# DCDmllm/AnyEdit

Hardware: NVIDIA H100
Metric: edited images/sec (512x512, 50-step DDIM, CFG) (higher is better)
Workload: dtype f16

## Files before the change

anyedit_b200/csrc/gemm_wgmma.cu:

```cuda
#include <cuda.h>
#include <stdlib.h>

#include "common.cuh"
#include "wgmma.cuh"

namespace anysd {

constexpr int G_BM = 128, G_BK = 64, G_THREADS = 384;
constexpr int G_A_BYTES = G_BM * G_BK * 2;

template <int BN>
struct GCfg {
    static constexpr int STAGE_BYTES = G_A_BYTES + BN * G_BK * 2;
    static constexpr int RED_BYTES = 8 * BN * 8;
    static constexpr int PAR_BYTES = 2 * 2 * BN * 4;
    static constexpr int FIT = (212 * 1024 - RED_BYTES - PAR_BYTES) / STAGE_BYTES;
    static constexpr int STAGES = FIT > 6 ? 6 : FIT;
    static constexpr int SMEM = STAGES * STAGE_BYTES + RED_BYTES + PAR_BYTES + 1024 + 256;
};

struct GArgs {
    const float* bias;
    const float* rowadd;
    const __half* residual;
    void* out;
    int M, N, ldo, ldr, ld_rowadd, rows_per_batch;
    int act, out_f16;
    int num_kb, tiles_m, tiles_n, num_tiles;
    int Nimg, Ho, Wo;
    int BW, BH, NB, tiles_w, tiles_h;
    int kb_per_tap, stride;
    int pad_lo;
    float* stats;
    int stats_hw, stats_spi, stats_nimg;
    int splits, kb_per_split, num_units;
    float* sk_ws;
    unsigned int* sk_cnt;
    float* row_stats;
    const float* ln_stats;
    const float* ln_colsum;
    int ln_slabs;
    float ln_eps, ln_inv_k;
};

__device__ __forceinline__ void g_bar_init(uint32_t bar, uint32_t count) {
    asm volatile("mbarrier.init.shared::cta.b64 [%0], %1;" ::"r"(bar), "r"(count));
}
__device__ __forceinline__ void g_expect_tx(uint32_t bar, uint32_t bytes) {
    asm volatile("mbarrier.arrive.expect_tx.shared::cta.b64 _, [%0], %1;" ::"r"(bar), "r"(bytes) : "memory");
}
__device__ __forceinline__ void g_arrive(uint32_t bar) {
    asm volatile("mbarrier.arrive.shared::cta.b64 _, [%0];" ::"r"(bar) : "memory");
}
__device__ __forceinline__ void g_wait(uint32_t bar, uint32_t parity) {
    asm volatile(
        "{\n\t"
        ".reg .pred P1;\n\t"
        "WAIT_LOOP:\n\t"
        "mbarrier.try_wait.parity.shared::cta.b64 P1, [%0], %1;\n\t"
        "@P1 bra DONE;\n\t"
        "bra WAIT_LOOP;\n\t"
        "DONE:\n\t"
        "}" ::"r"(bar), "r"(parity) : "memory");
}
__device__ __forceinline__ void g_tma_2d(uint32_t dst, const CUtensorMap* tm, uint32_t bar, int c0, int c1) {
    asm volatile("cp.async.bulk.tensor.2d.shared::cluster.global.mbarrier::complete_tx::bytes [%0], [%1, {%3, %4}], [%2];"
                 ::"r"(dst), "l"(tm), "r"(bar), "r"(c0), "r"(c1) : "memory");
}
__device__ __forceinline__ void g_tma_4d(uint32_t dst, const CUtensorMap* tm, uint32_t bar, int c0, int c1, int c2, int c3) {
    asm volatile("cp.async.bulk.tensor.4d.shared::cluster.global.mbarrier::complete_tx::bytes [%0], [%1, {%3, %4, %5, %6}], [%2];"
                 ::"r"(dst), "l"(tm), "r"(bar), "r"(c0), "r"(c1), "r"(c2), "r"(c3) : "memory");
}
__device__ __forceinline__ void g_pair_bar(int id) { asm volatile("bar.sync %0, 64;" ::"r"(id) : "memory"); }
__device__ __forceinline__ void g_wg_bar(int id) { asm volatile("bar.sync %0, 128;" ::"r"(id) : "memory"); }

__device__ __forceinline__ float p_gelu(float v) {
    const float t = fminf(v * v, 36.0f);
    float q = fmaf(t, 2.483638929e-05f, 7.36060983e-04f);
    q = fmaf(q, t, -0.10598272654f);
    q = fmaf(q, t, -2.30164716054f);
    float e, r;
    asm("ex2.approx.ftz.f32 %0, %1;" : "=f"(e) : "f"(v * q));
    asm("rcp.approx.ftz.f32 %0, %1;" : "=f"(r) : "f"(1.0f + e));
    return v * r;
}

struct TileCoord {
    int nt;
    int m0;
    int tw, th, tn;
};

template <bool CONV>
__device__ __forceinline__ TileCoord tile_coord(const GArgs& p, int tile) {
    TileCoord c;
    const int mt = tile / p.tiles_n;
    c.nt = tile - mt * p.tiles_n;
    c.m0 = mt * G_BM;
    c.tw = c.th = c.tn = 0;
    if (CONV) {
        c.tw = mt % p.tiles_w;
        c.th = (mt / p.tiles_w) % p.tiles_h;
        c.tn = mt / (p.tiles_w * p.tiles_h);
    }
    return c;
}

template <int BN, bool CONV>
__global__ void __launch_bounds__(G_THREADS, 1)
gemm_wgmma_kernel(const __grid_constant__ CUtensorMap tmA, const __grid_constant__ CUtensorMap tmB, const GArgs p) {
    using Cfg = GCfg<BN>;
    constexpr int STAGES = Cfg::STAGES;
    extern __shared__ unsigned char g_smem_raw[];
    const uint32_t raw = smem_u32(g_smem_raw);
    const uint32_t base = (raw + 1023u) & ~1023u;
    unsigned char* smem = g_smem_raw + (base - raw);
    float2* red = reinterpret_cast<float2*>(smem + STAGES * Cfg::STAGE_BYTES);
    float* par = reinterpret_cast<float*>(smem + STAGES * Cfg::STAGE_BYTES + Cfg::RED_BYTES);
    const uint32_t bars = base + STAGES * Cfg::STAGE_BYTES + Cfg::RED_BYTES + Cfg::PAR_BYTES;
    volatile int* sk_flag = reinterpret_cast<volatile int*>(smem + STAGES * Cfg::STAGE_BYTES + Cfg::RED_BYTES + Cfg::PAR_BYTES + 16 * STAGES);
    auto full_bar = [&](int s) { return bars + 8u * s; };
    auto empty_bar = [&](int s) { return bars + 8u * (STAGES + s); };
    const int warp = threadIdx.x >> 5, lane = threadIdx.x & 31;

    if (threadIdx.x == 0) {
        asm volatile("prefetch.tensormap [%0];" ::"l"(&tmA) : "memory");
        asm volatile("prefetch.tensormap [%0];" ::"l"(&tmB) : "memory");
        for (int s = 0; s < STAGES; ++s) {
            g_bar_init(full_bar(s), 1);
            g_bar_init(empty_bar(s), 8);
        }
        asm volatile("fence.mbarrier_init.release.cluster;" ::: "memory");
    }
    __syncthreads();

    if (warp < 4) {
        asm volatile("setmaxnreg.dec.sync.aligned.u32 40;" ::: "memory");
        if (warp == 0 && lane == 0) {
            uint32_t g = 0;
            for (int unit = blockIdx.x; unit < p.num_units; unit += gridDim.x) {
                const int tile = unit / p.splits;
                const int kb0 = (unit - tile * p.splits) * p.kb_per_split;
                const int kb1 = kb0 + p.kb_per_split < p.num_kb ? kb0 + p.kb_per_split : p.num_kb;
                const TileCoord c = tile_coord<CONV>(p, tile);
                const int n0 = c.nt * BN;
                for (int kb = kb0; kb < kb1; ++kb, ++g) {
                    const int s = g % STAGES;
                    g_wait(empty_bar(s), ((g / STAGES) & 1) ^ 1);
                    const uint32_t sa = base + s * Cfg::STAGE_BYTES, sb = sa + G_A_BYTES;
                    g_expect_tx(full_bar(s), Cfg::STAGE_BYTES);
                    if (CONV) {
                        const int tap = kb / p.kb_per_tap;
                        const int c0 = (kb - tap * p.kb_per_tap) * G_BK;
                        const int ky = tap / 3, kx = tap - ky * 3;
                        g_tma_4d(sa, &tmA, full_bar(s), c0, c.tw * p.BW * p.stride + kx - p.pad_lo,
                                 c.th * p.BH * p.stride + ky - p.pad_lo, c.tn * p.NB);
                    } else {
                        g_tma_2d(sa, &tmA, full_bar(s), kb * G_BK, c.m0);
                    }
                    g_tma_2d(sb, &tmB, full_bar(s), kb * G_BK, n0);
                }
            }
        }
        return;
    }

    asm volatile("setmaxnreg.inc.sync.aligned.u32 232;" ::: "memory");
    const int wg = (warp >> 2) - 1;
    const int wq = warp & 3;
    const int ew = wg * 4 + wq;
    const int slab = ew >> 1;
    const int rl0 = wg * 64 + wq * 16 + (lane >> 2);
    const int q4 = lane & 3;
    const bool ln_in = !CONV && p.ln_stats != nullptr;
    const bool row_st = !CONV && p.row_stats != nullptr;
    float* s_bias = par + wg * 2 * BN;
    float* s_cs = s_bias + BN;
    const int wtid = threadIdx.x & 127;
    float acc[BN / 2];
    uint32_t g = 0;
    for (int unit = blockIdx.x; unit < p.num_units; unit += gridDim.x) {
        const int tile = unit / p.splits;
        const int kb0 = (unit - tile * p.splits) * p.kb_per_split;
        const int kb1 = kb0 + p.kb_per_split < p.num_kb ? kb0 + p.kb_per_split : p.num_kb;
        const TileCoord c = tile_coord<CONV>(p, tile);
        const int n0 = c.nt * BN;
        float pb[2], pc[2];
#pragma unroll
        for (int r = 0; r < 2; ++r) {
            const int j = wtid + 128 * r, col = n0 + j;
            pb[r] = (j < BN && col < p.N && p.bias != nullptr) ? __ldg(p.bias + col) : 0.f;
            pc[r] = (j < BN && col < p.N && ln_in) ? __ldg(p.ln_colsum + col) : 0.f;
        }
#pragma unroll
        for (int i = 0; i < BN / 2; ++i) acc[i] = 0.f;
        for (int kb = kb0; kb < kb1; ++kb, ++g) {
            const int s = g % STAGES;
            g_wait(full_bar(s), (g / STAGES) & 1);
            const uint32_t sa = base + s * Cfg::STAGE_BYTES + wg * 64 * 128, sb = base + s * Cfg::STAGE_BYTES + G_A_BYTES;
            wg_fence();
#pragma unroll
            for (int k = 0; k < G_BK / 16; ++k) Wgmma<BN>::ss(acc, wg_desc(sa + 32 * k, 16, 1024), wg_desc(sb + 32 * k, 16, 1024), 1);
            wg_commit();
            wg_wait<1>();
            if (kb > kb0) {
                __syncwarp();
                if (lane == 0) g_arrive(empty_bar((g - 1) % STAGES));
            }
        }
        wg_wait<0>();
#pragma unroll
        for (int i = 0; i < BN / 2; ++i) wg_fence_regs(acc[i]);
        if (kb1 > kb0) {
            __syncwarp();
            if (lane == 0) g_arrive(empty_bar((g - 1) % STAGES));
        }
        g_wg_bar(5 + wg);
#pragma unroll
        for (int r = 0; r < 2; ++r) {
            if (wtid + 128 * r < BN) {
                s_bias[wtid + 128 * r] = pb[r];
                s_cs[wtid + 128 * r] = pc[r];
            }
        }
        g_wg_bar(5 + wg);

        if (p.splits > 1) {
            const int ks = unit - tile * p.splits;
            const float* wst = p.sk_ws + (size_t)tile * p.splits * (G_BM * BN);
            float* mine = p.sk_ws + ((size_t)tile * p.splits + ks) * (G_BM * BN);
#pragma unroll
            for (int i = 0; i < BN / 8; ++i)
#pragma unroll
                for (int h = 0; h < 2; ++h)
                    __stcg(reinterpret_cast<float2*>(mine + (size_t)(rl0 + 8 * h) * BN + 8 * i + 2 * q4),
                           make_float2(acc[4 * i + 2 * h], acc[4 * i + 2 * h + 1]));
            __threadfence();
            g_pair_bar(1 + slab);
            if ((ew & 1) == 0 && lane == 0) {
                unsigned int* cnt = p.sk_cnt + (size_t)tile * 4 + slab;
                const unsigned int old = atomicAdd(cnt, 1u);
                if (old == (unsigned)p.splits - 1) *cnt = 0;
                sk_flag[slab] = old == (unsigned)p.splits - 1;
            }
            g_pair_bar(1 + slab);
            const bool last = sk_flag[slab] != 0;
            g_pair_bar(1 + slab);
            if (!last) continue;
            __threadfence();
#pragma unroll
            for (int i = 0; i < BN / 2; ++i) acc[i] = 0.f;
            for (int k2 = 0; k2 < p.splits; ++k2) {
#pragma unroll
                for (int i = 0; i < BN / 8; ++i)
#pragma unroll
                    for (int h = 0; h < 2; ++h) {
                        const float2 f = __ldcg(reinterpret_cast<const float2*>(wst + (size_t)k2 * (G_BM * BN) +
                                                                                 (size_t)(rl0 + 8 * h) * BN + 8 * i + 2 * q4));
                        acc[4 * i + 2 * h] += f.x;
                        acc[4 * i + 2 * h + 1] += f.y;
                    }
            }
        }

        size_t pix[2];
        bool valid[2];
        int img[2];
        float ln_nm[2] = {0.f, 0.f}, ln_rs[2] = {1.f, 1.f};
#pragma unroll
        for (int h = 0; h < 2; ++h) {
            const int r = rl0 + 8 * h;
            if (CONV) {
                const int x = r % p.BW, y = (r / p.BW) % p.BH, n = r / (p.BW * p.BH);
                const int X = c.tw * p.BW + x, Y = c.th * p.BH + y, I = c.tn * p.NB + n;
                valid[h] = X < p.Wo && Y < p.Ho && I < p.Nimg;
                pix[h] = ((size_t)I * p.Ho + Y) * p.Wo + X;
                img[h] = I < p.Nimg ? I : p.Nimg - 1;
            } else {
                const int m = c.m0 + r;
                valid[h] = m < p.M;
                pix[h] = (size_t)m;
                img[h] = (m < p.M ? m : p.M - 1) / p.rows_per_batch;
                if (ln_in) {
                    const float2* sp2 = reinterpret_cast<const float2*>(p.ln_stats) + (m < p.M ? m : p.M - 1);
                    float s1 = 0.f, s2 = 0.f;
                    for (int sl = 0; sl < p.ln_slabs; ++sl) {
                        const float2 f = __ldg(sp2 + (size_t)sl * p.M);
                        s1 += f.x;
                        s2 += f.y;
                    }
                    const double mean = (double)s1 * (double)p.ln_inv_k;
                    double var = (double)s2 * (double)p.ln_inv_k - mean * mean;
                    if (var < 0.0) var = 0.0;
                    ln_nm[h] = -(float)mean;
                    ln_rs[h] = rsqrtf((float)var + p.ln_eps);
                }
            }
        }
        auto store2 = [&](int h, int ocol, float a, float b) {
            if (valid[h]) {
                if (p.residual != nullptr) {
                    const float2 r = __half22float2(*reinterpret_cast<const __half2*>(p.residual + pix[h] * p.ldr + ocol));
                    a += r.x;
                    b += r.y;
                }
                if (p.out_f16) *reinterpret_cast<__half2*>((__half*)p.out + pix[h] * p.ldo + ocol) = __floats2half2_rn(a, b);
                else *reinterpret_cast<float2*>((float*)p.out + pix[h] * p.ldo + ocol) = make_float2(a, b);
            }
        };

        float rs1[2] = {0.f, 0.f}, rs2[2] = {0.f, 0.f};
        constexpr int CH = 4;
        constexpr int UNROLL = BN <= 64 ? BN / 8 / CH : 1;
#pragma unroll UNROLL
        for (int i0 = 0; i0 < BN / 8; i0 += CH) {
            if (n0 + 8 * i0 >= p.N) break;
            float a[CH][4];
#pragma unroll
            for (int u = 0; u < CH; ++u)
#pragma unroll
                for (int e = 0; e < 4; ++e) a[u][e] = acc[4 * u + e];
#pragma unroll
            for (int k = CH; k < BN / 8; k += CH)
#pragma unroll
                for (int u = 0; u < CH; ++u)
#pragma unroll
                    for (int e = 0; e < 4; ++e) a[u][e] = k == i0 ? acc[4 * (k + u) + e] : a[u][e];
            float2 ra[CH][2];
            __half2 rr[CH][2];
#pragma unroll
            for (int u = 0; u < CH; ++u) {
                const int cw = n0 + 8 * (i0 + u) + 2 * q4;
                const bool in = cw < p.N;
#pragma unroll
                for (int h = 0; h < 2; ++h) {
                    ra[u][h] = (in && p.rowadd != nullptr)
                                   ? __ldg(reinterpret_cast<const float2*>(p.rowadd + (size_t)img[h] * p.ld_rowadd + cw))
                                   : make_float2(0.f, 0.f);
                    rr[u][h] = (in && valid[h] && p.residual != nullptr && p.act != 2)
                                   ? *reinterpret_cast<const __half2*>(p.residual + pix[h] * p.ldr + cw)
                                   : __floats2half2_rn(0.f, 0.f);
                }
            }
#pragma unroll
        for (int u = 0; u < CH; ++u) {
            const int i = i0 + u;
            if (n0 + 8 * i >= p.N) break;
            const int col = n0 + 8 * i + 2 * q4;
            float v[2][2];
            const float2 bb = *reinterpret_cast<const float2*>(s_bias + 8 * i + 2 * q4);
            if (ln_in) {
                const float2 cs = *reinterpret_cast<const float2*>(s_cs + 8 * i + 2 * q4);
#pragma unroll
                for (int h = 0; h < 2; ++h) {
                    v[h][0] = fmaf(ln_rs[h], fmaf(ln_nm[h], cs.x, a[u][2 * h]), bb.x);
                    v[h][1] = fmaf(ln_rs[h], fmaf(ln_nm[h], cs.y, a[u][2 * h + 1]), bb.y);
                }
            } else {
#pragma unroll
                for (int h = 0; h < 2; ++h) {
                    v[h][0] = a[u][2 * h] + bb.x;
                    v[h][1] = a[u][2 * h + 1] + bb.y;
                }
            }
#pragma unroll
            for (int h = 0; h < 2; ++h) {
                v[h][0] += ra[u][h].x;
                v[h][1] += ra[u][h].y;
            }
            if (p.act == 2) {
                float gv[2];
#pragma unroll
                for (int h = 0; h < 2; ++h) gv[h] = v[h][0] * (p.out_f16 ? p_gelu(v[h][1]) : gelu_erf_f(v[h][1]));
                const float recv = __shfl_xor_sync(0xffffffffu, (lane & 1) ? gv[0] : gv[1], 1);
                const int h = lane & 1;
                const int ocol = (col >> 1) - h;
                if (h) store2(1, ocol, recv, gv[1]);
                else store2(0, ocol, gv[0], recv);
                continue;
            }
            if (p.act != 0) {
#pragma unroll
                for (int h = 0; h < 2; ++h)
#pragma unroll
                    for (int e = 0; e < 2; ++e)
                        v[h][e] = p.act == 1 ? silu_f(v[h][e])
                                             : (p.act == 3 ? (p.out_f16 ? p_gelu(v[h][e]) : gelu_erf_f(v[h][e])) : quick_gelu_f(v[h][e]));
            }
#pragma unroll
            for (int h = 0; h < 2; ++h) {
                const float2 r = __half22float2(rr[u][h]);
                v[h][0] += r.x;
                v[h][1] += r.y;
                if (valid[h]) {
                    if (p.out_f16) *reinterpret_cast<__half2*>((__half*)p.out + pix[h] * p.ldo + col) = __floats2half2_rn(v[h][0], v[h][1]);
                    else *reinterpret_cast<float2*>((float*)p.out + pix[h] * p.ldo + col) = make_float2(v[h][0], v[h][1]);
                }
            }
            if (p.stats != nullptr) {
                float a0 = v[0][0] + v[1][0], a1 = v[0][1] + v[1][1];
                float b0 = v[0][0] * v[0][0] + v[1][0] * v[1][0], b1 = v[0][1] * v[0][1] + v[1][1] * v[1][1];
#pragma unroll
                for (int o = 4; o < 32; o <<= 1) {
                    a0 += __shfl_xor_sync(0xffffffffu, a0, o);
                    a1 += __shfl_xor_sync(0xffffffffu, a1, o);
                    b0 += __shfl_xor_sync(0xffffffffu, b0, o);
                    b1 += __shfl_xor_sync(0xffffffffu, b1, o);
                }
                if (lane < 4) {
                    red[ew * BN + 8 * i + 2 * lane] = make_float2(a0, b0);
                    red[ew * BN + 8 * i + 2 * lane + 1] = make_float2(a1, b1);
                }
            }
            if (row_st) {
#pragma unroll
                for (int h = 0; h < 2; ++h) {
                    rs1[h] += v[h][0] + v[h][1];
                    rs2[h] = fmaf(v[h][0], v[h][0], fmaf(v[h][1], v[h][1], rs2[h]));
                }
                if ((i & 7) == 7) {
#pragma unroll
                    for (int h = 0; h < 2; ++h) {
                        rs1[h] += __shfl_xor_sync(0xffffffffu, rs1[h], 1);
                        rs2[h] += __shfl_xor_sync(0xffffffffu, rs2[h], 1);
                        rs1[h] += __shfl_xor_sync(0xffffffffu, rs1[h], 2);
                        rs2[h] += __shfl_xor_sync(0xffffffffu, rs2[h], 2);
                        if (q4 == 0 && valid[h])
                            reinterpret_cast<float2*>(p.row_stats)[(size_t)((n0 >> 6) + (i >> 3)) * p.M + pix[h]] =
                                make_float2(rs1[h], rs2[h]);
                        rs1[h] = rs2[h] = 0.f;
                    }
                }
            }
        }
        }
        if (p.stats != nullptr) {
            g_pair_bar(1 + slab);
            if ((ew & 1) == 0) {
                int simg, sii;
                if (CONV) {
                    const int ppi = p.BW * p.BH;
                    simg = c.tn * p.NB + (slab * 32) / ppi;
                    sii = (c.th * p.tiles_w + c.tw) * (ppi >> 5) + (((slab * 32) % ppi) >> 5);
                } else {
                    const int r0 = c.m0 + slab * 32;
                    simg = r0 / p.stats_hw;
                    sii = (r0 - simg * p.stats_hw) >> 5;
                    if (r0 >= p.M) simg = p.stats_nimg;
                }
                if (simg < p.stats_nimg) {
                    for (int j = lane; j < BN && n0 + j < p.N; j += 32) {
                        const float2 x0 = red[ew * BN + j], x1 = red[(ew + 1) * BN + j];
                        reinterpret_cast<float2*>(p.stats)[((size_t)simg * p.stats_spi + sii) * p.N + n0 + j] =
                            make_float2(x0.x + x1.x, x0.y + x1.y);
                    }
                }
            }
            g_pair_bar(1 + slab);
        }
    }
}

typedef CUresult (*EncodeTiledFnP)(CUtensorMap*, CUtensorMapDataType, cuuint32_t, void*, const cuuint64_t*,
                                   const cuuint64_t*, const cuuint32_t*, const cuuint32_t*, CUtensorMapInterleave,
                                   CUtensorMapSwizzle, CUtensorMapL2promotion, CUtensorMapFloatOOBfill);
static EncodeTiledFnP p_get_encode() {
    static EncodeTiledFnP fn = nullptr;
    static bool tried = false;
    if (!tried) {
        tried = true;
        void* f = nullptr;
        cudaDriverEntryPointQueryResult qr;
        if (cudaGetDriverEntryPoint("cuTensorMapEncodeTiled", &f, cudaEnableDefault, &qr) == cudaSuccess &&
            qr == cudaDriverEntryPointSuccess)
            fn = (EncodeTiledFnP)f;
    }
    return fn;
}

struct PMapKey {
    const void* ptr;
    uint64_t d0, d1, d2, d3, ld;
    uint32_t b0, b1, b2, b3, es, rank;
    bool operator==(const PMapKey& o) const {
        return ptr == o.ptr && d0 == o.d0 && d1 == o.d1 && d2 == o.d2 && d3 == o.d3 && ld == o.ld && b0 == o.b0 && b1 == o.b1 &&
               b2 == o.b2 && b3 == o.b3 && es == o.es && rank == o.rank;
    }
};
struct PMapSlot {
    PMapKey key;
    CUtensorMap map;
    bool valid;
};
constexpr int P_MAP_SLOTS = 4096;
static thread_local PMapSlot* p_map_table = nullptr;
static PMapSlot* p_map_slot(const PMapKey& k) {
    if (p_map_table == nullptr) p_map_table = (PMapSlot*)calloc(P_MAP_SLOTS, sizeof(PMapSlot));
    uint64_t h = (uint64_t)(uintptr_t)k.ptr * 0x9E3779B97F4A7C15ull;
    h ^= (k.d0 * 31 + k.d1) * 0xC2B2AE3D27D4EB4Full + (k.d2 * 131 + k.d3 * 17 + k.ld) * 0x165667B19E3779F9ull;
    h ^= ((uint64_t)k.b0 << 40) ^ ((uint64_t)k.b1 << 28) ^ ((uint64_t)k.b2 << 16) ^ ((uint64_t)k.b3 << 4) ^ k.es ^ ((uint64_t)k.rank << 60);
    return p_map_table ? &p_map_table[(h >> 20) % P_MAP_SLOTS] : nullptr;
}

static bool p_map_2d(CUtensorMap* tm, const void* ptr, uint64_t inner, uint64_t outer, uint64_t ld, uint32_t bi, uint32_t bo) {
    const PMapKey key = {ptr, inner, outer, 0, 0, ld, bi, bo, 0, 0, 1, 2};
    PMapSlot* slot = p_map_slot(key);
    if (slot && slot->valid && slot->key == key) {
        *tm = slot->map;
        return true;
    }
    cuuint64_t dims[2] = {inner, outer};
    cuuint64_t strides[1] = {ld * 2};
    cuuint32_t box[2] = {bi, bo};
    cuuint32_t es[2] = {1, 1};
    const bool ok = p_get_encode()(tm, CU_TENSOR_MAP_DATA_TYPE_FLOAT16, 2, const_cast<void*>(ptr), dims, strides, box, es,
                                   CU_TENSOR_MAP_INTERLEAVE_NONE, CU_TENSOR_MAP_SWIZZLE_128B, CU_TENSOR_MAP_L2_PROMOTION_L2_256B,
                                   CU_TENSOR_MAP_FLOAT_OOB_FILL_NONE) == CUDA_SUCCESS;
    if (ok && slot) {
        slot->key = key;
        slot->map = *tm;
        slot->valid = true;
    }
    return ok;
}
static bool p_map_nhwc(CUtensorMap* tm, const void* ptr, int N, int H, int W, int C, int ld, int BW, int BH, int NB, int s) {
    const PMapKey key = {ptr, (uint64_t)C, (uint64_t)W, (uint64_t)H, (uint64_t)N, (uint64_t)ld, 64u, (uint32_t)BW, (uint32_t)BH, (uint32_t)NB,
                         (uint32_t)s, 4};
    PMapSlot* slot = p_map_slot(key);
    if (slot && slot->valid && slot->key == key) {
        *tm = slot->map;
        return true;
    }
    cuuint64_t dims[4] = {(cuuint64_t)C, (cuuint64_t)W, (cuuint64_t)H, (cuuint64_t)N};
    cuuint64_t strides[3] = {(cuuint64_t)ld * 2, (cuuint64_t)W * ld * 2, (cuuint64_t)H * W * ld * 2};
    cuuint32_t box[4] = {64u, (cuuint32_t)(BW * s), (cuuint32_t)(BH * s), (cuuint32_t)NB};
    cuuint32_t es[4] = {1, (cuuint32_t)s, (cuuint32_t)s, 1};
    const bool ok = p_get_encode()(tm, CU_TENSOR_MAP_DATA_TYPE_FLOAT16, 4, const_cast<void*>(ptr), dims, strides, box, es,
                                   CU_TENSOR_MAP_INTERLEAVE_NONE, CU_TENSOR_MAP_SWIZZLE_128B, CU_TENSOR_MAP_L2_PROMOTION_L2_256B,
                                   CU_TENSOR_MAP_FLOAT_OOB_FILL_NONE) == CUDA_SUCCESS;
    if (ok && slot) {
        slot->key = key;
        slot->map = *tm;
        slot->valid = true;
    }
    return ok;
}

static int p_pow2_ceil(int v) {
    int r = 1;
    while (r < v) r <<= 1;
    return r;
}
static int p_pick_extent(int len, int cap) {
    int lim = p_pow2_ceil(len);
    if (lim > cap) lim = cap;
    for (int c = lim; c >= 4; c >>= 1)
        if (len % c == 0) return c;
    return lim;
}

__global__ void upsample2x_kernel(const uint4* __restrict__ src, uint4* __restrict__ dst, int H, int W, int CV, long long total) {
    for (long long i = blockIdx.x * (long long)blockDim.x + threadIdx.x; i < total; i += (long long)gridDim.x * blockDim.x) {
        const int cv = (int)(i % CV);
        long long r = i / CV;
        const int ox = (int)(r % (2 * W));
        r /= (2 * W);
        const int oy = (int)(r % (2 * H));
        const long long n = r / (2 * H);
        dst[i] = __ldg(src + ((n * H + (oy >> 1)) * W + (ox >> 1)) * CV + cv);
    }
}

int launch_upsample2x(const __half* src, __half* dst, int N, int H, int W, int C, cudaStream_t st) {
    const long long total = (long long)N * 4 * H * W * (C / 8);
    int grid = (int)((total + 255) / 256);
    if (grid > sm_count() * 16) grid = sm_count() * 16;
    upsample2x_kernel<<<grid, 256, 0, st>>>((const uint4*)src, (uint4*)dst, H, W, C / 8, total);
    return check_launch("upsample2x");
}

static void p_conv_patch(const anysd_gemm_params* q, int* Ho, int* Wo, int* BW, int* BH, int* NB) {
    const int Hin = q->H << q->upsample, Win = q->Wd << q->upsample;
    *Ho = q->conv_pad ? (Hin - 2) / 2 + 1 : (Hin - 1) / q->stride + 1;
    *Wo = q->conv_pad ? (Win - 2) / 2 + 1 : (Win - 1) / q->stride + 1;
    *BW = p_pick_extent(*Wo, 128);
    *BH = p_pick_extent(*Ho, 128 / *BW);
    *NB = 128 / (*BW * *BH);
}

int wg_stats_slabs(const anysd_gemm_params* q) {
    if (q->act == 2 || q->out_dtype != ANYSD_F16) return 0;
    const int hw = q->rows_per_batch;
    if (hw <= 0 || hw % 32 != 0 || q->M % hw != 0) return 0;
    if (q->conv) {
        int Ho, Wo, BW, BH, NB;
        p_conv_patch(q, &Ho, &Wo, &BW, &BH, &NB);
        if (Ho * Wo != hw || (BW * BH) % 32 != 0 || Wo % BW != 0 || Ho % BH != 0) return 0;
    }
    return hw / 32;
}

static int p_geometry_splits(const anysd_gemm_params* q, int num_kb) {
    static const char* force_sk = getenv("ANYSD_GEMM_SPLITK");
    if (q->act == 2 || q->out_dtype != ANYSD_F16 || q->row_stats != nullptr || q->ln_stats != nullptr) return 1;
    int rows_per_image = q->rows_per_batch;
    if (q->conv) {
        int Ho, Wo, BW, BH, NB;
        p_conv_patch(q, &Ho, &Wo, &BW, &BH, &NB);
        rows_per_image = Ho * Wo;
    }
    if (rows_per_image <= 0 || rows_per_image > G_BM) return 1;
    if (force_sk) {
        const int f = atoi(force_sk);
        return (f <= 1 || num_kb / f < 8) ? 1 : (f > 8 ? 8 : f);
    }
    return (q->conv && num_kb >= 256) ? 3 : 1;
}

static void p_select(const anysd_gemm_params* q, int tiles_m, int num_kb, int* bn_out, int* splits_out) {
    static const char* force_bn = getenv("ANYSD_GEMM_BN");
    const int sp = splits_out ? p_geometry_splits(q, num_kb) : 1;
    int bn = 256;
    double best = -1;
    static const int widths[4] = {256, 192, 128, 64};
    for (int wi = 0; wi < 4; ++wi) {
        const int w = widths[wi];
        if (force_bn && atoi(force_bn) != w) continue;
        const long units = (long)tiles_m * cdiv(q->N, w) * sp;
        const long slots = sm_count();
        const long rounds = (units + slots - 1) / slots;
        const double cost = (double)rounds * (w + 270) * ((double)cdiv(num_kb, sp) + (sp > 1 ? 8.0 : 0.0));
        if (best < 0 || cost < best) { best = cost; bn = w; }
    }
    *bn_out = bn;
    if (splits_out) *splits_out = sp;
}
static size_t p_splitk_bytes(int tiles_m, int N, int bn, int splits) {
    if (splits <= 1) return 0;
    return (size_t)tiles_m * cdiv(N, bn) * splits * G_BM * bn * sizeof(float);
}

static void p_tiles(const anysd_gemm_params* q, int* tiles_m, int* num_kb) {
    if (q->conv) {
        int Ho, Wo, BW, BH, NB;
        p_conv_patch(q, &Ho, &Wo, &BW, &BH, &NB);
        *tiles_m = cdiv(Wo, BW) * cdiv(Ho, BH) * cdiv(q->Nimg, NB);
        *num_kb = 9 * (q->Cin / G_BK);
    } else {
        *tiles_m = cdiv(q->M, G_BM);
        *num_kb = cdiv(q->K, G_BK);
    }
}

size_t wg_splitk_bytes(const anysd_gemm_params* q) {
    int tiles_m, num_kb, bn, splits;
    p_tiles(q, &tiles_m, &num_kb);
    p_select(q, tiles_m, num_kb, &bn, &splits);
    return p_splitk_bytes(tiles_m, q->N, bn, splits);
}

static const char* wg_ln_unsupported(const anysd_gemm_params* q) {
    if (q->conv) return "dense contractions only";
    if (q->out_dtype != ANYSD_F16) return "fp16 output only";
    if (q->row_stats != nullptr) {
        if (q->act != 0) return "row statistics need act = 0";
        if (q->N % 64 != 0) return "row statistics need N % 64 == 0";
        if ((uintptr_t)q->row_stats % 8) return "row_stats must be 8-byte aligned";
    }
    if (q->ln_stats != nullptr) {
        if (q->K % 64 != 0) return "folded LayerNorm needs K % 64 == 0";
        if (q->bias == nullptr || q->ln_colsum == nullptr) return "folded LayerNorm needs bias (beta W^T + b) and ln_colsum";
        if (((uintptr_t)q->ln_stats % 8) || ((uintptr_t)q->ln_colsum % 16)) return "ln_stats / ln_colsum misaligned";
        if (q->N % 32 != 0) return "folded LayerNorm needs N % 32 == 0";
        if (q->act != 0 && q->act != 1 && q->act != 2) return "folded LayerNorm: act must be 0, 1 or 2";
    }
    return nullptr;
}

bool wg_supported(const anysd_gemm_params* q) {
    if (q->N % 8 != 0 || q->K % 8 != 0) return false;
    if (q->act == 2 && q->N % 16 != 0) return false;
    const int n_out = q->act == 2 ? q->N / 2 : q->N;
    if (((uintptr_t)q->out % 16) || q->ldo % 8 != 0 || n_out % 4 != 0) return false;
    if (q->residual && (((uintptr_t)q->residual % 16) || q->ldr % 8 != 0)) return false;
    if (q->bias && ((uintptr_t)q->bias % 16)) return false;
    if (q->rowadd && (((uintptr_t)q->rowadd % 16) || q->ld_rowadd % 4 != 0)) return false;
    if (q->conv) {
        if (q->Cin % G_BK != 0) return false;
        if (q->upsample) {
            const size_t need = (size_t)q->Nimg * (2 * q->H) * (2 * q->Wd) * q->Cin * sizeof(__half);
            if (q->workspace == nullptr || q->workspace_bytes < need || ((uintptr_t)q->workspace % 16)) return false;
        }
    }
    return p_get_encode() != nullptr;
}

template <int BN, bool CONV>
static int p_launch(const CUtensorMap& tmA, const CUtensorMap& tmB, const GArgs& a, cudaStream_t st) {
    static bool done[64];
    int dev = 0;
    cudaGetDevice(&dev);
    dev &= 63;
    if (!done[dev]) {
        cudaError_t e = cudaFuncSetAttribute(gemm_wgmma_kernel<BN, CONV>, cudaFuncAttributeMaxDynamicSharedMemorySize, GCfg<BN>::SMEM);
        if (e != cudaSuccess) {
            set_error("wgmma gemm: smem opt-in failed: %s", cudaGetErrorString(e));
            return ANYSD_ECUDA;
        }
        done[dev] = true;
    }
    int grid = sm_count();
    if (grid > a.num_units) grid = a.num_units;
    gemm_wgmma_kernel<BN, CONV><<<grid, G_THREADS, GCfg<BN>::SMEM, st>>>(tmA, tmB, a);
    return check_launch(CONV ? "conv3x3 (wgmma)" : "gemm (wgmma)");
}

template <bool CONV>
static int p_launch_bn(int bn, const CUtensorMap& tmA, const CUtensorMap& tmB, const GArgs& a, cudaStream_t st) {
    switch (bn) {
        case 256: return p_launch<256, CONV>(tmA, tmB, a, st);
        case 192: return p_launch<192, CONV>(tmA, tmB, a, st);
        case 128: return p_launch<128, CONV>(tmA, tmB, a, st);
        default: return p_launch<64, CONV>(tmA, tmB, a, st);
    }
}

int launch_gemm_wg(const anysd_gemm_params* q, cudaStream_t st) {
    GArgs a;
    a.stats = nullptr;
    a.stats_hw = a.stats_spi = a.stats_nimg = 0;
    if (q->stats != nullptr) {
        a.stats_spi = wg_stats_slabs(q);
        if (a.stats_spi == 0 || q->stats_images <= 0) {
            set_error("gemm: output statistics requested for a shape that cannot produce them (M=%d rows_per_batch=%d conv=%d act=%d); "
                      "query anysd_gemm_stats_slabs first", q->M, q->rows_per_batch, q->conv, q->act);
            return ANYSD_EUNSUPPORTED;
        }
        a.stats = q->stats;
        a.stats_hw = q->rows_per_batch;
        a.stats_nimg = q->stats_images;
    }
    a.row_stats = q->row_stats;
    a.ln_stats = q->ln_stats;
    a.ln_colsum = q->ln_colsum;
    a.ln_slabs = q->K / 64;
    a.ln_eps = q->ln_eps;
    a.ln_inv_k = 1.0f / (float)q->K;
    if (q->row_stats != nullptr || q->ln_stats != nullptr) {
        const char* why = wg_ln_unsupported(q);
        if (why) {
            set_error("gemm: LayerNorm fold / row statistics: %s (M=%d N=%d K=%d act=%d)", why, q->M, q->N, q->K, q->act);
            return ANYSD_EUNSUPPORTED;
        }
        if (q->stats != nullptr || q->act >= 3) {
            set_error("gemm: LayerNorm fold / row statistics cannot be combined with GroupNorm statistics or GELU epilogues");
            return ANYSD_EUNSUPPORTED;
        }
    }
    a.bias = q->bias;
    a.rowadd = q->rowadd;
    a.residual = (const __half*)q->residual;
    a.out = q->out;
    a.M = q->M;
    a.N = q->N;
    a.ldo = q->ldo;
    a.ldr = q->ldr;
    a.ld_rowadd = q->ld_rowadd;
    a.rows_per_batch = q->rows_per_batch > 0 ? q->rows_per_batch : 1;
    a.act = q->act;
    a.out_f16 = q->out_dtype == ANYSD_F16;
    a.Nimg = q->Nimg;
    a.BW = a.BH = a.NB = a.tiles_w = a.tiles_h = 1;
    a.kb_per_tap = 1;
    a.stride = q->conv ? q->stride : 1;
    a.pad_lo = (q->conv && q->conv_pad) ? 0 : 1;
    a.Ho = a.Wo = 0;
    CUtensorMap tmA, tmB;
    bool ok = true;
    p_tiles(q, &a.tiles_m, &a.num_kb);
    if (q->conv) {
        const void* img = q->A;
        int Hin = q->H, Win = q->Wd;
        if (q->upsample) {
            int rc = launch_upsample2x((const __half*)q->A, (__half*)q->workspace, q->Nimg, q->H, q->Wd, q->Cin, st);
            if (rc) return rc;
            img = q->workspace;
            Hin *= 2;
            Win *= 2;
        }
        p_conv_patch(q, &a.Ho, &a.Wo, &a.BW, &a.BH, &a.NB);
        a.tiles_w = cdiv(a.Wo, a.BW);
        a.tiles_h = cdiv(a.Ho, a.BH);
        a.kb_per_tap = q->Cin / G_BK;
        ok = ok && p_map_nhwc(&tmA, img, q->Nimg, Hin, Win, q->Cin, q->Cin, a.BW, a.BH, a.NB, a.stride);
    } else {
        ok = ok && p_map_2d(&tmA, q->A, (uint64_t)q->K, (uint64_t)q->M, (uint64_t)q->lda, G_BK, G_BM);
    }
    int bn = 256, splits = 1;
    p_select(q, a.tiles_m, a.num_kb, &bn, &splits);
    const size_t sk_need = p_splitk_bytes(a.tiles_m, q->N, bn, splits);
    if (splits > 1 && (q->splitk_workspace == nullptr || q->splitk_workspace_bytes < sk_need || q->splitk_counters == nullptr ||
                       (size_t)a.tiles_m * cdiv(q->N, bn) * 4 * sizeof(unsigned int) > q->splitk_counters_bytes)) {
        splits = 1;
        p_select(q, a.tiles_m, a.num_kb, &bn, nullptr);
    }
    a.tiles_n = cdiv(q->N, bn);
    ok = ok && p_map_2d(&tmB, q->W, (uint64_t)q->K, (uint64_t)q->N, (uint64_t)q->ldw, G_BK, bn);
    if (!ok) {
        set_error("wgmma gemm: cuTensorMapEncodeTiled failed (M=%d N=%d K=%d conv=%d)", q->M, q->N, q->K, q->conv);
        return ANYSD_ECUDA;
    }
    a.num_tiles = a.tiles_m * a.tiles_n;
    a.splits = splits;
    a.kb_per_split = cdiv(a.num_kb, splits);
    a.num_units = a.num_tiles * splits;
    a.sk_ws = (float*)q->splitk_workspace;
    a.sk_cnt = (unsigned int*)q->splitk_counters;
    return q->conv ? p_launch_bn<true>(bn, tmA, tmB, a, st) : p_launch_bn<false>(bn, tmA, tmB, a, st);
}

}
```

Measured before the change: 3.634.

## Add ping-pong warpgroup GEMM kernel for short-K non-conv GEMMs

Adds a 128x128 ping-pong kernel in which two consumer warpgroups take alternate tiles and hand off the MMA turn through named barriers. Each warpgroup's epilogue, which stages output through per-warp shared memory with coalesced 16-byte stores and cp.async residual loads, overlaps the other warpgroup's mainloop. The selector routes non-conv GEMMs with at most 10 K-blocks and at least two tiles per SM to this kernel. The aim is to hide epilogue cost on short-K GEMMs, at the cost of more complexity and a larger shared-memory footprint that may reduce pipeline stages.

```diff
diff --git a/anyedit_b200/csrc/gemm_wgmma.cu b/anyedit_b200/csrc/gemm_wgmma.cu
--- a/anyedit_b200/csrc/gemm_wgmma.cu
+++ b/anyedit_b200/csrc/gemm_wgmma.cu
@@ -8,15 +8,19 @@
 
 constexpr int G_BM = 128, G_BK = 64, G_THREADS = 384;
 constexpr int G_A_BYTES = G_BM * G_BK * 2;
+constexpr int G_OUT_PITCH_MAX = 160, G_RES_PITCH = 80;
+constexpr int G_STG_WARP = 16 * G_OUT_PITCH_MAX + 16 * G_RES_PITCH + 16 * 8;
 
 template <int BN>
-struct GCfg {
+struct GPingCfg {
+    static_assert(BN == 128, "ping-pong tiles are 128 x 128");
     static constexpr int STAGE_BYTES = G_A_BYTES + BN * G_BK * 2;
     static constexpr int RED_BYTES = 8 * BN * 8;
     static constexpr int PAR_BYTES = 2 * 2 * BN * 4;
-    static constexpr int FIT = (212 * 1024 - RED_BYTES - PAR_BYTES) / STAGE_BYTES;
+    static constexpr int STG_BYTES = 8 * G_STG_WARP;
+    static constexpr int FIT = (212 * 1024 - RED_BYTES - PAR_BYTES - STG_BYTES) / STAGE_BYTES;
     static constexpr int STAGES = FIT > 6 ? 6 : FIT;
-    static constexpr int SMEM = STAGES * STAGE_BYTES + RED_BYTES + PAR_BYTES + 1024 + 256;
+    static constexpr int SMEM = STAGES * STAGE_BYTES + RED_BYTES + PAR_BYTES + STG_BYTES + 1024 + 256;
 };
 
 struct GArgs {
@@ -73,6 +77,8 @@
 }
 __device__ __forceinline__ void g_pair_bar(int id) { asm volatile("bar.sync %0, 64;" ::"r"(id) : "memory"); }
 __device__ __forceinline__ void g_wg_bar(int id) { asm volatile("bar.sync %0, 128;" ::"r"(id) : "memory"); }
+__device__ __forceinline__ void g_turn_wait(int id) { asm volatile("bar.sync %0, 256;" ::"r"(id) : "memory"); }
+__device__ __forceinline__ void g_turn_pass(int id) { asm volatile("bar.arrive %0, 256;" ::"r"(id) : "memory"); }
 
 __device__ __forceinline__ float p_gelu(float v) {
     const float t = fminf(v * v, 36.0f);
@@ -106,10 +112,26 @@
     return c;
 }
 
+__device__ __forceinline__ void unit_kb(const GArgs& p, int unit, int& tile, int& kb0, int& kb1) {
+    tile = unit / p.splits;
+    kb0 = (unit - tile * p.splits) * p.kb_per_split;
+    kb1 = kb0 + p.kb_per_split < p.num_kb ? kb0 + p.kb_per_split : p.num_kb;
+}
+
+template <int BN>
+struct GCoopCfg {
+    static constexpr int STAGE_BYTES = G_A_BYTES + BN * G_BK * 2;
+    static constexpr int RED_BYTES = 8 * BN * 8;
+    static constexpr int PAR_BYTES = 2 * 2 * BN * 4;
+    static constexpr int FIT = (212 * 1024 - RED_BYTES - PAR_BYTES) / STAGE_BYTES;
+    static constexpr int STAGES = FIT > 6 ? 6 : FIT;
+    static constexpr int SMEM = STAGES * STAGE_BYTES + RED_BYTES + PAR_BYTES + 1024 + 256;
+};
+
 template <int BN, bool CONV>
 __global__ void __launch_bounds__(G_THREADS, 1)
-gemm_wgmma_kernel(const __grid_constant__ CUtensorMap tmA, const __grid_constant__ CUtensorMap tmB, const GArgs p) {
-    using Cfg = GCfg<BN>;
+gemm_coop_kernel(const __grid_constant__ CUtensorMap tmA, const __grid_constant__ CUtensorMap tmB, const GArgs p) {
+    using Cfg = GCoopCfg<BN>;
     constexpr int STAGES = Cfg::STAGES;
     extern __shared__ unsigned char g_smem_raw[];
     const uint32_t raw = smem_u32(g_smem_raw);
@@ -461,6 +483,369 @@
     }
 }
 
+template <int BN, bool CONV>
+__global__ void __launch_bounds__(G_THREADS, 1)
+gemm_pingpong_kernel(const __grid_constant__ CUtensorMap tmA, const __grid_constant__ CUtensorMap tmB, const GArgs p) {
+    using Cfg = GPingCfg<BN>;
+    constexpr int STAGES = Cfg::STAGES;
+    extern __shared__ unsigned char g_smem_raw[];
+    const uint32_t raw = smem_u32(g_smem_raw);
+    const uint32_t base = (raw + 1023u) & ~1023u;
+    unsigned char* smem = g_smem_raw + (base - raw);
+    unsigned char* tail = smem + STAGES * Cfg::STAGE_BYTES;
+    float2* red = reinterpret_cast<float2*>(tail);
+    float* par = reinterpret_cast<float*>(tail + Cfg::RED_BYTES);
+    unsigned char* stg = tail + Cfg::RED_BYTES + Cfg::PAR_BYTES;
+    const uint32_t bars = base + STAGES * Cfg::STAGE_BYTES + Cfg::RED_BYTES + Cfg::PAR_BYTES + Cfg::STG_BYTES;
+        auto full_bar = [&](int s) { return bars + 8u * s; };
+    auto empty_bar = [&](int s) { return bars + 8u * (STAGES + s); };
+    const int warp = threadIdx.x >> 5, lane = threadIdx.x & 31;
+
+    if (threadIdx.x == 0) {
+        asm volatile("prefetch.tensormap [%0];" ::"l"(&tmA) : "memory");
+        asm volatile("prefetch.tensormap [%0];" ::"l"(&tmB) : "memory");
+        for (int s = 0; s < STAGES; ++s) {
+            g_bar_init(full_bar(s), 1);
+            g_bar_init(empty_bar(s), 4);
+        }
+        asm volatile("fence.mbarrier_init.release.cluster;" ::: "memory");
+    }
+    __syncthreads();
+
+    if (warp < 4) {
+        asm volatile("setmaxnreg.dec.sync.aligned.u32 40;" ::: "memory");
+        if (warp == 0 && lane == 0) {
+            uint32_t g = 0;
+            for (int unit = blockIdx.x; unit < p.num_units; unit += gridDim.x) {
+                int tile, kb0, kb1;
+                unit_kb(p, unit, tile, kb0, kb1);
+                const TileCoord c = tile_coord<CONV>(p, tile);
+                const int n0 = c.nt * BN;
+                for (int kb = kb0; kb < kb1; ++kb, ++g) {
+                    const int s = g % STAGES;
+                    g_wait(empty_bar(s), ((g / STAGES) & 1) ^ 1);
+                    const uint32_t sa = base + s * Cfg::STAGE_BYTES, sb = sa + G_A_BYTES;
+                    g_expect_tx(full_bar(s), Cfg::STAGE_BYTES);
+                    if (CONV) {
+                        const int tap = kb / p.kb_per_tap;
+                        const int c0 = (kb - tap * p.kb_per_tap) * G_BK;
+                        const int ky = tap / 3, kx = tap - ky * 3;
+                        g_tma_4d(sa, &tmA, full_bar(s), c0, c.tw * p.BW * p.stride + kx - p.pad_lo,
+                                 c.th * p.BH * p.stride + ky - p.pad_lo, c.tn * p.NB);
+                    } else {
+                        g_tma_2d(sa, &tmA, full_bar(s), kb * G_BK, c.m0);
+                    }
+                    g_tma_2d(sb, &tmB, full_bar(s), kb * G_BK, n0);
+                }
+            }
+        }
+        return;
+    }
+
+    asm volatile("setmaxnreg.inc.sync.aligned.u32 232;" ::: "memory");
+    const int wg = (warp >> 2) - 1;
+    const int wq = warp & 3;
+    const int ew = wg * 4 + wq;
+    const int pair = 1 + 2 * wg + (wq >> 1);
+    const int q4 = lane & 3;
+    const bool ln_in = !CONV && p.ln_stats != nullptr;
+    const bool row_st = !CONV && p.row_stats != nullptr;
+    const bool geglu = p.act == 2;
+    const int n_out = geglu ? p.N >> 1 : p.N;
+    const int oes = p.out_f16 ? 2 : 4;
+    const int opitch = p.out_f16 ? 144 : 160;
+    float* s_bias = par + wg * 2 * BN;
+    float* s_cs = s_bias + BN;
+    unsigned char* s_out = stg + ew * G_STG_WARP;
+    __half* s_res = reinterpret_cast<__half*>(s_out + 16 * G_OUT_PITCH_MAX);
+    long long* s_pix = reinterpret_cast<long long*>(s_out + 16 * G_OUT_PITCH_MAX + 16 * G_RES_PITCH);
+    const int wtid = threadIdx.x & 127;
+    float acc[BN];
+    uint32_t g = 0;
+    if (wg == 1) {
+        int tile, kb0, kb1;
+        unit_kb(p, blockIdx.x, tile, kb0, kb1);
+        g += kb1 - kb0;
+    }
+    for (int unit = blockIdx.x + wg * gridDim.x; unit < p.num_units; unit += 2 * gridDim.x) {
+        int tile, kb0, kb1;
+        unit_kb(p, unit, tile, kb0, kb1);
+        const TileCoord c = tile_coord<CONV>(p, tile);
+        const int n0 = c.nt * BN;
+        float pb[2], pc[2];
+#pragma unroll
+        for (int r = 0; r < 2; ++r) {
+            const int j = wtid + 128 * r, col = n0 + j;
+            pb[r] = (j < BN && col < p.N && p.bias != nullptr) ? __ldg(p.bias + col) : 0.f;
+            pc[r] = (j < BN && col < p.N && ln_in) ? __ldg(p.ln_colsum + col) : 0.f;
+        }
+#pragma unroll
+        for (int i = 0; i < BN; ++i) acc[i] = 0.f;
+        if (unit != (int)blockIdx.x) g_turn_wait(7 + wg);
+        for (int kb = kb0; kb < kb1; ++kb, ++g) {
+            const int s = g % STAGES;
+            g_wait(full_bar(s), (g / STAGES) & 1);
+            const uint32_t sa = base + s * Cfg::STAGE_BYTES, sb = sa + G_A_BYTES;
+            wg_fence();
+#pragma unroll
+            for (int k = 0; k < G_BK / 16; ++k)
+#pragma unroll
+                for (int h2 = 0; h2 < 2; ++h2)
+                    Wgmma<BN>::ss(acc + h2 * (BN / 2), wg_desc(sa + h2 * 64 * 128 + 32 * k, 16, 1024), wg_desc(sb + 32 * k, 16, 1024), 1);
+            wg_commit();
+            wg_wait<1>();
+            if (kb > kb0) {
+                __syncwarp();
+                if (lane == 0) g_arrive(empty_bar((g - 1) % STAGES));
+            }
+        }
+        const uint32_t g_last = g - 1;
+        if (unit + (int)gridDim.x < p.num_units) {
+            g_turn_pass(7 + (wg ^ 1));
+            int t2, k0, k1;
+            unit_kb(p, unit + gridDim.x, t2, k0, k1);
+            g += k1 - k0;
+        }
+        wg_wait<0>();
+#pragma unroll
+        for (int i = 0; i < BN; ++i) wg_fence_regs(acc[i]);
+        if (kb1 > kb0) {
+            __syncwarp();
+            if (lane == 0) g_arrive(empty_bar(g_last % STAGES));
+        }
+        g_wg_bar(5 + wg);
+#pragma unroll
+        for (int r = 0; r < 2; ++r) {
+            if (wtid + 128 * r < BN) {
+                s_bias[wtid + 128 * r] = pb[r];
+                s_cs[wtid + 128 * r] = pc[r];
+            }
+        }
+        g_wg_bar(5 + wg);
+
+#pragma unroll 1
+        for (int h2 = 0; h2 < 2; ++h2) {
+            const int rl0 = 64 * h2 + 16 * wq + (lane >> 2);
+            size_t pix[2];
+            bool valid[2];
+            int img[2];
+            float ln_nm[2] = {0.f, 0.f}, ln_rs[2] = {1.f, 1.f};
+#pragma unroll
+            for (int h = 0; h < 2; ++h) {
+                const int r = rl0 + 8 * h;
+                if (CONV) {
+                    const int x = r % p.BW, y = (r / p.BW) % p.BH, n = r / (p.BW * p.BH);
+                    const int X = c.tw * p.BW + x, Y = c.th * p.BH + y, I = c.tn * p.NB + n;
+                    valid[h] = X < p.Wo && Y < p.Ho && I < p.Nimg;
+                    pix[h] = ((size_t)I * p.Ho + Y) * p.Wo + X;
+                    img[h] = I < p.Nimg ? I : p.Nimg - 1;
+                } else {
+                    const int m = c.m0 + r;
+                    valid[h] = m < p.M;
+                    pix[h] = (size_t)m;
+                    img[h] = (m < p.M ? m : p.M - 1) / p.rows_per_batch;
+                    if (ln_in) {
+                        const float2* sp2 = reinterpret_cast<const float2*>(p.ln_stats) + (m < p.M ? m : p.M - 1);
+                        float s1 = 0.f, s2 = 0.f;
+                        for (int sl = 0; sl < p.ln_slabs; ++sl) {
+                            const float2 f = __ldg(sp2 + (size_t)sl * p.M);
+                            s1 += f.x;
+                            s2 += f.y;
+                        }
+                        const double mean = (double)s1 * (double)p.ln_inv_k;
+                        double var = (double)s2 * (double)p.ln_inv_k - mean * mean;
+                        if (var < 0.0) var = 0.0;
+                        ln_nm[h] = -(float)mean;
+                        ln_rs[h] = rsqrtf((float)var + p.ln_eps);
+                    }
+                }
+            }
+            if (q4 == 0) {
+                s_pix[lane >> 2] = valid[0] ? (long long)pix[0] : -1ll;
+                s_pix[(lane >> 2) + 8] = valid[1] ? (long long)pix[1] : -1ll;
+            }
+            __syncwarp();
+
+            float rs1[2] = {0.f, 0.f}, rs2[2] = {0.f, 0.f};
+            constexpr int CH = 4;
+            constexpr int UNROLL = BN <= 64 ? BN / 8 / CH : 1;
+#pragma unroll UNROLL
+            for (int i0 = 0; i0 < BN / 8; i0 += CH) {
+                if (n0 + 8 * i0 >= p.N) break;
+                const int ob = geglu ? (n0 + 8 * i0) >> 1 : n0 + 8 * i0;
+                if (p.residual != nullptr) {
+                    const int rsh = geglu ? 1 : 2;
+#pragma unroll
+                    for (int t2 = 0; t2 < 2; ++t2) {
+                        const int t = lane + 32 * t2, r = t >> rsh, vi = t & ((1 << rsh) - 1), oc = ob + 8 * vi;
+                        if (r < 16) {
+                            const long long px = s_pix[r];
+                            const bool in = px >= 0 && oc < n_out;
+                            cp_async16(smem_u32(s_res + r * (G_RES_PITCH / 2) + 8 * vi),
+                                       in ? p.residual + (size_t)px * p.ldr + oc : p.residual, in);
+                        }
+                    }
+                    cp_async_commit();
+                }
+                float a[CH][4];
+                const int kk = h2 * (BN / 8) + i0;
+#pragma unroll
+                for (int u = 0; u < CH; ++u)
+#pragma unroll
+                    for (int e = 0; e < 4; ++e) a[u][e] = acc[4 * u + e];
+#pragma unroll
+                for (int k = CH; k < BN / 4; k += CH)
+#pragma unroll
+                    for (int u = 0; u < CH; ++u)
+#pragma unroll
+                        for (int e = 0; e < 4; ++e) a[u][e] = k == kk ? acc[4 * (k + u) + e] : a[u][e];
+                if (p.residual != nullptr) {
+                    cp_async_wait<0>();
+                    __syncwarp();
+                }
+                auto put = [&](int h, int oc, float x, float y) {
+                    const int r = (lane >> 2) + 8 * h;
+                    if (p.residual != nullptr) {
+                        const float2 rr = __half22float2(*reinterpret_cast<const __half2*>(s_res + r * (G_RES_PITCH / 2) + oc));
+                        x += rr.x;
+                        y += rr.y;
+                    }
+                    if (p.out_f16) *reinterpret_cast<__half2*>(s_out + r * opitch + 2 * oc) = __floats2half2_rn(x, y);
+                    else *reinterpret_cast<float2*>(s_out + r * opitch + 4 * oc) = make_float2(x, y);
+                    return make_float2(x, y);
+                };
+#pragma unroll
+                for (int u = 0; u < CH; ++u) {
+                    const int i = i0 + u;
+                    if (n0 + 8 * i >= p.N) break;
+                    float v[2][2];
+                    const float2 bb = *reinterpret_cast<const float2*>(s_bias + 8 * i + 2 * q4);
+                    if (ln_in) {
+                        const float2 cs = *reinterpret_cast<const float2*>(s_cs + 8 * i + 2 * q4);
+#pragma unroll
+                        for (int h = 0; h < 2; ++h) {
+                            v[h][0] = fmaf(ln_rs[h], fmaf(ln_nm[h], cs.x, a[u][2 * h]), bb.x);
+                            v[h][1] = fmaf(ln_rs[h], fmaf(ln_nm[h], cs.y, a[u][2 * h + 1]), bb.y);
+                        }
+                    } else {
+#pragma unroll
+                        for (int h = 0; h < 2; ++h) {
+                            v[h][0] = a[u][2 * h] + bb.x;
+                            v[h][1] = a[u][2 * h + 1] + bb.y;
+                        }
+                    }
+                    if (p.rowadd != nullptr) {
+#pragma unroll
+                        for (int h = 0; h < 2; ++h) {
+                            const float2 ra = __ldg(reinterpret_cast<const float2*>(p.rowadd + (size_t)img[h] * p.ld_rowadd + n0 + 8 * i + 2 * q4));
+                            v[h][0] += ra.x;
+                            v[h][1] += ra.y;
+                        }
+                    }
+                    if (geglu) {
+                        float gv[2];
+#pragma unroll
+                        for (int h = 0; h < 2; ++h) gv[h] = v[h][0] * (p.out_f16 ? p_gelu(v[h][1]) : gelu_erf_f(v[h][1]));
+                        const float recv = __shfl_xor_sync(0xffffffffu, (lane & 1) ? gv[0] : gv[1], 1);
+                        const int h = lane & 1;
+                        const int oc = 4 * u + q4 - h;
+                        if (h) put(1, oc, recv, gv[1]);
+                        else put(0, oc, gv[0], recv);
+                        continue;
+                    }
+                    if (p.act != 0) {
+#pragma unroll
+                        for (int h = 0; h < 2; ++h)
+#pragma unroll
+                            for (int e = 0; e < 2; ++e)
+                                v[h][e] = p.act == 1 ? silu_f(v[h][e])
+                                                     : (p.act == 3 ? (p.out_f16 ? p_gelu(v[h][e]) : gelu_erf_f(v[h][e])) : quick_gelu_f(v[h][e]));
+                    }
+#pragma unroll
+                    for (int h = 0; h < 2; ++h) {
+                        const float2 w = put(h, 8 * u + 2 * q4, v[h][0], v[h][1]);
+                        v[h][0] = w.x;
+                        v[h][1] = w.y;
+                    }
+                    if (p.stats != nullptr) {
+                        float a0 = v[0][0] + v[1][0], a1 = v[0][1] + v[1][1];
+                        float b0 = v[0][0] * v[0][0] + v[1][0] * v[1][0], b1 = v[0][1] * v[0][1] + v[1][1] * v[1][1];
+#pragma unroll
+                        for (int o = 4; o < 32; o <<= 1) {
+                            a0 += __shfl_xor_sync(0xffffffffu, a0, o);
+                            a1 += __shfl_xor_sync(0xffffffffu, a1, o);
+                            b0 += __shfl_xor_sync(0xffffffffu, b0, o);
+                            b1 += __shfl_xor_sync(0xffffffffu, b1, o);
+                        }
+                        if (lane < 4) {
+                            red[ew * BN + 8 * i + 2 * lane] = make_float2(a0, b0);
+                            red[ew * BN + 8 * i + 2 * lane + 1] = make_float2(a1, b1);
+                        }
+                    }
+                    if (row_st) {
+#pragma unroll
+                        for (int h = 0; h < 2; ++h) {
+                            rs1[h] += v[h][0] + v[h][1];
+                            rs2[h] = fmaf(v[h][0], v[h][0], fmaf(v[h][1], v[h][1], rs2[h]));
+                        }
+                        if ((i & 7) == 7) {
+#pragma unroll
+                            for (int h = 0; h < 2; ++h) {
+                                rs1[h] += __shfl_xor_sync(0xffffffffu, rs1[h], 1);
+                                rs2[h] += __shfl_xor_sync(0xffffffffu, rs2[h], 1);
+                                rs1[h] += __shfl_xor_sync(0xffffffffu, rs1[h], 2);
+                                rs2[h] += __shfl_xor_sync(0xffffffffu, rs2[h], 2);
+                                const long long px = s_pix[(lane >> 2) + 8 * h];
+                                if (q4 == 0 && px >= 0)
+                                    reinterpret_cast<float2*>(p.row_stats)[(size_t)((n0 >> 6) + (i >> 3)) * p.M + px] =
+                                        make_float2(rs1[h], rs2[h]);
+                                rs1[h] = rs2[h] = 0.f;
+                            }
+                        }
+                    }
+                }
+                __syncwarp();
+                const int vsh = (geglu ? 0 : 1) + (p.out_f16 ? 1 : 2);
+                const int epv = 16 / oes;
+                for (int t = lane; t < (16 << vsh); t += 32) {
+                    const int r = t >> vsh, vi = t & ((1 << vsh) - 1), oc = ob + vi * epv;
+                    const long long px = s_pix[r];
+                    if (px >= 0 && oc < n_out)
+                        *reinterpret_cast<uint4*>(static_cast<unsigned char*>(p.out) + ((size_t)px * p.ldo + oc) * oes) =
+                            *reinterpret_cast<const uint4*>(s_out + r * opitch + 16 * vi);
+                }
+                __syncwarp();
+            }
+            if (p.stats != nullptr) {
+                const int slab = 2 * h2 + (wq >> 1);
+                g_pair_bar(pair);
+                if ((wq & 1) == 0) {
+                    int simg, sii;
+                    if (CONV) {
+                        const int ppi = p.BW * p.BH;
+                        simg = c.tn * p.NB + (slab * 32) / ppi;
+                        sii = (c.th * p.tiles_w + c.tw) * (ppi >> 5) + (((slab * 32) % ppi) >> 5);
+                    } else {
+                        const int r0 = c.m0 + slab * 32;
+                        simg = r0 / p.stats_hw;
+                        sii = (r0 - simg * p.stats_hw) >> 5;
+                        if (r0 >= p.M) simg = p.stats_nimg;
+                    }
+                    if (simg < p.stats_nimg) {
+                        for (int j = lane; j < BN && n0 + j < p.N; j += 32) {
+                            const float2 x0 = red[ew * BN + j], x1 = red[(ew + 1) * BN + j];
+                            reinterpret_cast<float2*>(p.stats)[((size_t)simg * p.stats_spi + sii) * p.N + n0 + j] =
+                                make_float2(x0.x + x1.x, x0.y + x1.y);
+                        }
+                    }
+                }
+                g_pair_bar(pair);
+            }
+            __syncwarp();
+        }
+    }
+}
+
 typedef CUresult (*EncodeTiledFnP)(CUtensorMap*, CUtensorMapDataType, cuuint32_t, void*, const cuuint64_t*,
                                    const cuuint64_t*, const cuuint32_t*, const cuuint32_t*, CUtensorMapInterleave,
                                    CUtensorMapSwizzle, CUtensorMapL2promotion, CUtensorMapFloatOOBfill);
@@ -617,9 +1002,17 @@
     return (q->conv && num_kb >= 256) ? 3 : 1;
 }
 
-static void p_select(const anysd_gemm_params* q, int tiles_m, int num_kb, int* bn_out, int* splits_out) {
+static void p_select(const anysd_gemm_params* q, int tiles_m, int num_kb, int* bn_out, int* splits_out, bool* pingpong_out) {
     static const char* force_bn = getenv("ANYSD_GEMM_BN");
     const int sp = splits_out ? p_geometry_splits(q, num_kb) : 1;
+    const bool pingpong = !q->conv && sp == 1 && num_kb <= 10 && (long)tiles_m * cdiv(q->N, 128) >= 2L * sm_count() &&
+                          (!force_bn || atoi(force_bn) == 128);
+    if (pingpong_out) *pingpong_out = pingpong;
+    if (splits_out) *splits_out = sp;
+    if (pingpong) {
+        *bn_out = 128;
+        return;
+    }
     int bn = 256;
     double best = -1;
     static const int widths[4] = {256, 192, 128, 64};
@@ -633,7 +1026,6 @@
         if (best < 0 || cost < best) { best = cost; bn = w; }
     }
     *bn_out = bn;
-    if (splits_out) *splits_out = sp;
 }
 static size_t p_splitk_bytes(int tiles_m, int N, int bn, int splits) {
     if (splits <= 1) return 0;
@@ -655,7 +1047,7 @@
 size_t wg_splitk_bytes(const anysd_gemm_params* q) {
     int tiles_m, num_kb, bn, splits;
     p_tiles(q, &tiles_m, &num_kb);
-    p_select(q, tiles_m, num_kb, &bn, &splits);
+    p_select(q, tiles_m, num_kb, &bn, &splits, nullptr);
     return p_splitk_bytes(tiles_m, q->N, bn, splits);
 }
 
@@ -695,14 +1087,23 @@
     return p_get_encode() != nullptr;
 }
 
-template <int BN, bool CONV>
+template <int BN, bool CONV, bool PINGPONG>
 static int p_launch(const CUtensorMap& tmA, const CUtensorMap& tmB, const GArgs& a, cudaStream_t st) {
     static bool done[64];
+    int smem;
+    void (*kernel)(const CUtensorMap, const CUtensorMap, const GArgs);
+    if constexpr (PINGPONG) {
+        smem = GPingCfg<BN>::SMEM;
+        kernel = gemm_pingpong_kernel<BN, CONV>;
+    } else {
+        smem = GCoopCfg<BN>::SMEM;
+        kernel = gemm_coop_kernel<BN, CONV>;
+    }
     int dev = 0;
     cudaGetDevice(&dev);
     dev &= 63;
     if (!done[dev]) {
-        cudaError_t e = cudaFuncSetAttribute(gemm_wgmma_kernel<BN, CONV>, cudaFuncAttributeMaxDynamicSharedMemorySize, GCfg<BN>::SMEM);
+        cudaError_t e = cudaFuncSetAttribute(kernel, cudaFuncAttributeMaxDynamicSharedMemorySize, smem);
         if (e != cudaSuccess) {
             set_error("wgmma gemm: smem opt-in failed: %s", cudaGetErrorString(e));
             return ANYSD_ECUDA;
@@ -711,17 +1112,17 @@
     }
     int grid = sm_count();
     if (grid > a.num_units) grid = a.num_units;
-    gemm_wgmma_kernel<BN, CONV><<<grid, G_THREADS, GCfg<BN>::SMEM, st>>>(tmA, tmB, a);
+    kernel<<<grid, G_THREADS, smem, st>>>(tmA, tmB, a);
     return check_launch(CONV ? "conv3x3 (wgmma)" : "gemm (wgmma)");
 }
 
 template <bool CONV>
 static int p_launch_bn(int bn, const CUtensorMap& tmA, const CUtensorMap& tmB, const GArgs& a, cudaStream_t st) {
     switch (bn) {
-        case 256: return p_launch<256, CONV>(tmA, tmB, a, st);
-        case 192: return p_launch<192, CONV>(tmA, tmB, a, st);
-        case 128: return p_launch<128, CONV>(tmA, tmB, a, st);
-        default: return p_launch<64, CONV>(tmA, tmB, a, st);
+        case 256: return p_launch<256, CONV, false>(tmA, tmB, a, st);
+        case 192: return p_launch<192, CONV, false>(tmA, tmB, a, st);
+        case 128: return p_launch<128, CONV, false>(tmA, tmB, a, st);
+        default: return p_launch<64, CONV, false>(tmA, tmB, a, st);
     }
 }
 
@@ -797,12 +1198,13 @@
         ok = ok && p_map_2d(&tmA, q->A, (uint64_t)q->K, (uint64_t)q->M, (uint64_t)q->lda, G_BK, G_BM);
     }
     int bn = 256, splits = 1;
-    p_select(q, a.tiles_m, a.num_kb, &bn, &splits);
+    bool pingpong = false;
+    p_select(q, a.tiles_m, a.num_kb, &bn, &splits, &pingpong);
     const size_t sk_need = p_splitk_bytes(a.tiles_m, q->N, bn, splits);
     if (splits > 1 && (q->splitk_workspace == nullptr || q->splitk_workspace_bytes < sk_need || q->splitk_counters == nullptr ||
                        (size_t)a.tiles_m * cdiv(q->N, bn) * 4 * sizeof(unsigned int) > q->splitk_counters_bytes)) {
         splits = 1;
-        p_select(q, a.tiles_m, a.num_kb, &bn, nullptr);
+        p_select(q, a.tiles_m, a.num_kb, &bn, nullptr, &pingpong);
     }
     a.tiles_n = cdiv(q->N, bn);
     ok = ok && p_map_2d(&tmB, q->W, (uint64_t)q->K, (uint64_t)q->N, (uint64_t)q->ldw, G_BK, bn);
@@ -816,6 +1218,7 @@
     a.num_units = a.num_tiles * splits;
     a.sk_ws = (float*)q->splitk_workspace;
     a.sk_cnt = (unsigned int*)q->splitk_counters;
+    if (pingpong) return p_launch<128, false, true>(tmA, tmB, a, st);
     return q->conv ? p_launch_bn<true>(bn, tmA, tmB, a, st) : p_launch_bn<false>(bn, tmA, tmB, a, st);
 }
 
```

Result: faster. 3.777 (median of 6 runs) (+3.9%).
